# megvii-research/AAAI2023-PVD

Hardware: AMD Instinct MI355X
Metric: train rays/s (hash->vm chair distillation step) (higher is better)
Workload: dtype f16 tables+MLP (AMP, as the reference forces) / f32 marcher+compositor; 1 GPU; distill hash->vm, synthetic chair, synthetic cameras, stage 3 (rgb + feature/sigma/colour losses), 4096 rays/GPU/step, occupancy 128^3 5.0% occupied, max_steps 1024, teacher pre-trained 300 steps; rays_per_gpu=4096, parallelism=ray-dp1, update=AdamW in one launch, capture_fallback=False

## Files before the change

aaai2023-pvd_amd/csrc/raymarching.hip:

```cpp
#include "dda.h"
#include "rays.h"

#include <float.h>

namespace pvd {

constexpr uint32_t kBlock = 256;
constexpr float kRPi = 0.3183098861837907f;


__global__ void __launch_bounds__(kBlock) k_near_far(const float *__restrict__ rays_o, const float *__restrict__ rays_d,
                                                     const float *__restrict__ aabb, uint32_t N, float min_near,
                                                     float *__restrict__ nears, float *__restrict__ fars) {
    const uint32_t n = blockIdx.x * kBlock + threadIdx.x;
    if (n >= N) return;
    const float o[3] = {rays_o[3 * (size_t)n], rays_o[3 * (size_t)n + 1], rays_o[3 * (size_t)n + 2]};
    const float d[3] = {rays_d[3 * (size_t)n], rays_d[3 * (size_t)n + 1], rays_d[3 * (size_t)n + 2]};
    near_far_of(o, d, aabb, min_near, nears[n], fars[n]);
}

__global__ void __launch_bounds__(kBlock) k_polar(const float *__restrict__ rays_o, const float *__restrict__ rays_d,
                                                  float radius, uint32_t N, float *__restrict__ coords) {
    const uint32_t n = blockIdx.x * kBlock + threadIdx.x;
    if (n >= N) return;
    const float ox = rays_o[3 * (size_t)n], oy = rays_o[3 * (size_t)n + 1], oz = rays_o[3 * (size_t)n + 2];
    const float dx = rays_d[3 * (size_t)n], dy = rays_d[3 * (size_t)n + 1], dz = rays_d[3 * (size_t)n + 2];
    const float A = dx * dx + dy * dy + dz * dz;
    const float Bh = ox * dx + oy * dy + oz * dz;
    const float Cc = ox * ox + oy * oy + oz * oz - radius * radius;
    const float t = (-Bh + sqrtf(Bh * Bh - A * Cc)) / A;
    const float x = ox + t * dx, y = oy + t * dy, z = oz + t * dz;
    const float theta = atan2f(sqrtf(x * x + z * z), y);
    const float phi = atan2f(z, x);
    coords[2 * (size_t)n] = 2 * theta * kRPi - 1;
// ... 254 lines not shown
            const uint32_t n_before = emitted - (uint32_t)__popcll(emit_mask);
            const int prev_lane = below ? 63 - __clzll((long long)below) : 0;
            const float prev_after = __shfl(t_after, prev_lane, 64);
            if ((emit_mask >> lane) & 1ull) {
                const size_t k = n_before + (uint32_t)__popcll(below);
                xyzs[3 * k] = x; xyzs[3 * k + 1] = y; xyzs[3 * k + 2] = z;
                dirs[3 * k] = r.dx; dirs[3 * k + 1] = r.dy; dirs[3 * k + 2] = r.dz;
                deltas[2 * k] = dtp;
                deltas[2 * k + 1] = t_after - (below ? prev_after : last_t);
            }
            last_t = readlane_f(t_after, 63u - (uint32_t)__clzll((long long)emit_mask));
        }
        if (rec && emit_mask) {
            if (rec->n < kMarchMaxRecords) {
                if (lane == 0) { rec->chunk[rec->n].mask = emit_mask; rec->chunk[rec->n].t_base = t_base; }
                rec->n++;
            } else {
                rec->overflow = true;
            }
        }
        if (done) break;
        t_base = readlane_f(t_after, 63);
        if (!fast && !grows) {
            const uint32_t b61 = __float_as_uint(readlane_f(t_after, 61)), b62 = __float_as_uint(readlane_f(t_after, 62));
            const uint32_t b63 = __float_as_uint(t_base);
            lat_c = ((b61 >> 23) == (b63 >> 23) && (b62 >> 23) == (b63 >> 23)) ? b63 - b62 : 0u;
        }
    }
    return emitted;
}

constexpr uint32_t kRaysPerBlock = kBlock / kWave;

__global__ void __launch_bounds__(kBlock) k_march_count_wave(const float *__restrict__ rays_o, const float *__restrict__ rays_d,
                                                             const uint8_t *__restrict__ grid, float bound, float dt_gamma, uint32_t max_steps,
                                                             uint32_t N, uint32_t C, uint32_t H, const float *__restrict__ nears,
                                                             const float *__restrict__ fars, int32_t *__restrict__ rays, uint32_t perturb,
                                                             MarchRayRecords *__restrict__ records, const int32_t *__restrict__ counter,
                                                             uint32_t fresh) {
    if (records && blockIdx.x == 0 && threadIdx.x == 0) records[N].n = fresh ? 0u : (uint32_t)counter[0];
    const uint32_t n = blockIdx.x * kRaysPerBlock + (threadIdx.x >> 6);
    const uint32_t lane = threadIdx.x & 63u;
    if (n >= N) return;
#ifdef PVD_MARCH_PROFILE
    const long long prof_t0 = __builtin_readcyclecounter();
    uint32_t prof_chunks = 0;
#endif
    Dda r;
    r.init(rays_o + 3 * (size_t)n, rays_d + 3 * (size_t)n, bound, dt_gamma, max_steps, C, H, grid);
    const float t0 = ray_t0(nears[n], r.dt_min, perturb, 42u, n);
    const float far = fars[n];
    uint32_t num;
    if (t0 >= 0.0f && t0 < far) {
        MarchRecord rec = {records ? records[n].chunk : nullptr, 0u, false};
#ifdef PVD_MARCH_PROFILE
        num = march_ray_wave<false>(r, t0, far, max_steps, lane, nullptr, nullptr, nullptr, &prof_chunks, records ? &rec : nullptr);
#else
        num = march_ray_wave<false>(r, t0, far, max_steps, lane, nullptr, nullptr, nullptr, nullptr, records ? &rec : nullptr);
#endif
        if (records && lane == 0) { records[n].n = rec.n; records[n].overflow = rec.overflow ? 1u : 0u; }
    } else {
        float t = t0;
        num = 0;
        while (t < far && num < max_steps) {
            float x, y, z, dt, tn;
            if (r.probe(t, x, y, z, dt, tn)) { num++; t += dt; }
            else t = tn;
        }
        if (records && lane == 0) { records[n].n = 0; records[n].overflow = num ? 1u : 0u; }
    }
    if (lane == 0) rays[3 * (size_t)n + 2] = (int32_t)num;
#ifdef PVD_MARCH_PROFILE
    if (lane == 0) { rays[3 * (size_t)n] = (int32_t)(__builtin_readcyclecounter() - prof_t0); rays[3 * (size_t)n + 1] = (int32_t)prof_chunks; }
#endif
}

__global__ void __launch_bounds__(kBlock) k_march_write_wave(const float *__restrict__ rays_o, const float *__restrict__ rays_d,
                                                             const uint8_t *__restrict__ grid, float bound, float dt_gamma, uint32_t max_steps,
                                                             uint32_t N, uint32_t C, uint32_t H, uint32_t M,
                                                             const float *__restrict__ nears, const float *__restrict__ fars,
                                                             float *__restrict__ xyzs, float *__restrict__ dirs, float *__restrict__ deltas,
                                                             const int32_t *__restrict__ rays, uint32_t perturb,
                                                             const int32_t *__restrict__ budget) {
    const uint32_t n = blockIdx.x * kRaysPerBlock + (threadIdx.x >> 6);
    const uint32_t lane = threadIdx.x & 63u;
    if (n >= N) return;
// ... 672 lines not shown

int pvd_morton3D_invert(const int32_t *indices, uint32_t N, int32_t *coords, pvd_stream_t stream) {
    if (N == 0) return PVD_OK;
    PVD_REQUIRE(coords && indices);
    hipLaunchKernelGGL(k_morton3D_invert, dim3(div_up(N, kBlock)), dim3(kBlock), 0, (hipStream_t)stream, indices, N, coords);
    return check_launch();
}

int pvd_packbits(const float *grid, uint32_t N, float density_thresh, uint8_t *bitfield, pvd_stream_t stream) {
    if (N == 0) return PVD_OK;
    PVD_REQUIRE(grid && bitfield);
    PVD_REQUIRE((reinterpret_cast<uintptr_t>(grid) & 15u) == 0);
    hipLaunchKernelGGL(k_packbits, dim3(div_up(N, kBlock)), dim3(kBlock), 0, (hipStream_t)stream, grid, N, density_thresh, bitfield);
    return check_launch();
}

constexpr uint32_t kMarchFusedScanMaxRays = 16384;

size_t pvd_march_workspace_bytes(uint32_t N) { return ((size_t)N + 1) * sizeof(MarchRayRecords); }

int pvd_march_rays_train(const float *rays_o, const float *rays_d, const uint8_t *grid, float bound, float dt_gamma,
                         uint32_t max_steps, uint32_t N, uint32_t C, uint32_t H, uint32_t M, const float *nears,
                         const float *fars, float *xyzs, float *dirs, float *deltas, int32_t *rays, int32_t *counter,
                         uint32_t perturb, pvd_stream_t stream) {
    return pvd_march_rays_train_ws(rays_o, rays_d, grid, bound, dt_gamma, max_steps, N, C, H, M, nears, fars, xyzs, dirs, deltas, rays,
                                   counter, perturb, nullptr, 0, 0u, nullptr, stream);
}

int pvd_march_rays_train_ws(const float *rays_o, const float *rays_d, const uint8_t *grid, float bound, float dt_gamma,
                            uint32_t max_steps, uint32_t N, uint32_t C, uint32_t H, uint32_t M, const float *nears,
                            const float *fars, float *xyzs, float *dirs, float *deltas, int32_t *rays, int32_t *counter,
                            uint32_t perturb, void *workspace, size_t workspace_bytes, uint32_t flags, const int32_t *budget_dev,
                            pvd_stream_t stream) {
    hipStream_t s = (hipStream_t)stream;
    const bool fresh = (flags & PVD_MARCH_FRESH) != 0;
    if (N == 0) {
        if (fresh && M && xyzs && dirs && deltas && counter) {
            (void)hipMemsetAsync(xyzs, 0, 3 * (size_t)M * sizeof(float), s); (void)hipMemsetAsync(dirs, 0, 3 * (size_t)M * sizeof(float), s);
            (void)hipMemsetAsync(deltas, 0, 2 * (size_t)M * sizeof(float), s); (void)hipMemsetAsync(counter, 0, 2 * sizeof(int32_t), s);
        }
        return PVD_OK;
    }
    PVD_REQUIRE(rays_o && rays_d && grid && nears && fars && xyzs && dirs && deltas && rays && counter);
    PVD_REQUIRE(C >= 1 && C <= 16 && H >= 1 && H <= 1024 && max_steps >= 1);
    MarchRayRecords *records = (workspace && workspace_bytes >= pvd_march_workspace_bytes(N) && N <= kMarchFusedScanMaxRays)
                                   ? (MarchRayRecords *)workspace : nullptr;
    if (fresh && !records) {
        (void)hipMemsetAsync(xyzs, 0, 3 * (size_t)M * sizeof(float), s); (void)hipMemsetAsync(dirs, 0, 3 * (size_t)M * sizeof(float), s);
        (void)hipMemsetAsync(deltas, 0, 2 * (size_t)M * sizeof(float), s); (void)hipMemsetAsync(counter, 0, 2 * sizeof(int32_t), s);
    }
    const dim3 g(div_up(N, kRaysPerBlock)), b(kBlock);
    hipLaunchKernelGGL(k_march_count_wave, g, b, 0, s, rays_o, rays_d, grid, bound, dt_gamma, max_steps, N, C, H, nears, fars, rays, perturb,
                       records, counter, records && fresh ? 1u : 0u);
    if (records) {
        hipLaunchKernelGGL(k_march_write_records, g, b, 0, s, rays_o, rays_d, grid, bound, dt_gamma, max_steps, N, C, H, M, nears, fars, xyzs,
                           dirs, deltas, rays, perturb, records, counter, fresh ? 1u : 0u, budget_dev);
        return check_launch();
    }
#ifdef PVD_MARCH_PROFILE
    return check_launch();
#endif
    hipLaunchKernelGGL(k_march_scan, dim3(1), dim3(kScanBlock), 0, s, rays, N, counter);
    hipLaunchKernelGGL(k_march_write_wave, g, b, 0, s, rays_o, rays_d, grid, bound, dt_gamma, max_steps, N, C, H, M, nears, fars, xyzs, dirs,
                       deltas, rays, perturb, budget_dev);
    return check_launch();
}

int pvd_composite_rays_train_forward(const float *sigmas, const float *rgbs, const float *deltas, const int32_t *rays,
                                     uint32_t M, uint32_t N, float *weights_sum, float *depth, float *image,
                                     pvd_stream_t stream) {
    if (N == 0) return PVD_OK;
    PVD_REQUIRE(sigmas && rgbs && deltas && rays && weights_sum && depth && image);
    hipLaunchKernelGGL(k_composite_fwd_wave<false>, dim3(div_up(N, kBlock / kWave)), dim3(kBlock), 0, (hipStream_t)stream, sigmas, rgbs, deltas,
                       rays, M, N, weights_sum, depth, image, CompositeEpilogue{});
    return check_launch();
}

int pvd_composite_rays_train_backward(const float *grad_weights_sum, const float *grad_image, const float *sigmas,
                                      const float *rgbs, const float *deltas, const int32_t *rays, const float *weights_sum,
                                      const float *image, uint32_t M, uint32_t N, float *grad_sigmas, float *grad_rgbs,
                                      pvd_stream_t stream) {
    if (N == 0) return PVD_OK;
    PVD_REQUIRE(grad_weights_sum && grad_image && sigmas && rgbs && deltas && rays && weights_sum && image && grad_sigmas && grad_rgbs);
    hipLaunchKernelGGL(k_composite_bwd_wave<false>, dim3(div_up(N, kBlock / kWave)), dim3(kBlock), 0, (hipStream_t)stream, grad_weights_sum,
                       grad_image, sigmas, rgbs, deltas, rays, weights_sum, image, M, N, grad_sigmas, grad_rgbs, CompositeEpilogue{});
    return check_launch();
// ... 162 lines not shown
```

aaai2023-pvd_amd/pvd/renderer.py:

```python
import math

import numpy as np
import torch
import torch.nn as nn


def near_far_from_aabb_torch(rays_o, rays_d, aabb, min_near):
    rd = 1.0 / rays_d
    lo = (aabb[:3] - rays_o) * rd
    hi = (aabb[3:] - rays_o) * rd
    t_lo, t_hi = torch.minimum(lo, hi), torch.maximum(lo, hi)
    near, far = t_lo[:, 0], t_hi[:, 0]
    miss = torch.zeros_like(near, dtype=torch.bool)
    for a in (1, 2):
        miss = miss | (near > t_hi[:, a]) | (t_lo[:, a] > far)
        near, far = torch.maximum(near, t_lo[:, a]), torch.minimum(far, t_hi[:, a])
    big = torch.finfo(near.dtype).max
    near = torch.where(miss, torch.full_like(near, big), near.clamp_min(min_near))
    far = torch.where(miss, torch.full_like(far, big), far)
    return near, far


def sample_pdf(bins, weights, n_samples, det=False):
    pdf = weights + 1e-5
# ... 8 lines not shown
    hi = torch.searchsorted(cdf, u, right=True)
    lo = (hi - 1).clamp_min(0)
    hi = hi.clamp_max(cdf.shape[-1] - 1)
    c_lo, c_hi = torch.gather(cdf, -1, lo), torch.gather(cdf, -1, hi)
    b_lo, b_hi = torch.gather(bins, -1, lo), torch.gather(bins, -1, hi)
    width = c_hi - c_lo
    width = torch.where(width < 1e-5, torch.ones_like(width), width)
    return b_lo + (u - c_lo) / width * (b_hi - b_lo)


class NeRFRenderer(nn.Module):
    def __init__(self, ops, bound=1, cuda_ray=True, density_scale=1, min_near=0.2, density_thresh=0.01, bg_radius=-1,
                 grid_size=128, teacher_variant=False):
        super().__init__()
        self.ops = ops
        self.rm = ops.raymarching
        self.bound = bound
        self.cascade = 1 + math.ceil(math.log2(bound))
        self.grid_size = grid_size
        self.density_scale = density_scale
        self.min_near = min_near
        self.density_thresh = density_thresh
        self.bg_radius = bg_radius
        self.teacher_variant = teacher_variant

        aabb = torch.FloatTensor([-bound, -bound, -bound, bound, bound, bound])
        self.register_buffer("aabb_train", aabb)
        self.register_buffer("aabb_infer", aabb.clone())

        self.cuda_ray = cuda_ray
        if cuda_ray:
            self.register_buffer("density_grid", torch.zeros([self.cascade, grid_size ** 3]))
            self.register_buffer("density_bitfield", torch.zeros(self.cascade * grid_size ** 3 // 8, dtype=torch.uint8))
            self.mean_density = 0
            self.iter_density = 0
            self.register_buffer("step_counter", torch.zeros(16, 2, dtype=torch.int32))
            self.mean_count = 0
            self.local_step = 0
        if bg_radius > 0:
            raise NotImplementedError("bg_radius > 0 (background model) is not supported: the reference's own branch asserts out "
                                      "(distill_mutual/network.py:496)")
        self.occ_epoch = 0

    def note_occupancy_changed(self):
        self.occ_epoch += 1

    def load_state_dict(self, state_dict, strict=True, **kw):
        out = super().load_state_dict(state_dict, strict=strict, **kw)
        self.note_occupancy_changed()
        return out

    def forward(self, x, d):
        raise NotImplementedError()

    def density(self, x):
        raise NotImplementedError()

    def reset_extra_state(self):
        if not self.cuda_ray:
            return
        self.density_grid.zero_()
        self.note_occupancy_changed()
        self.mean_density = 0
        self.iter_density = 0
        self.step_counter.zero_()
        self.mean_count = 0
        self.local_step = 0

    def run(self, rays_o, rays_d, num_steps=128, upsample_steps=128, bg_color=None, perturb=False, **kwargs):
        prefix = rays_o.shape[:-1]
        rays_o = rays_o.contiguous().view(-1, 3)
        rays_d = rays_d.contiguous().view(-1, 3)
        N, device = rays_o.shape[0], rays_o.device
        aabb = self.aabb_train if self.training else self.aabb_infer
        nears, fars = near_far_from_aabb_torch(rays_o, rays_d, aabb, self.min_near)
        nears, fars = nears.unsqueeze(-1), fars.unsqueeze(-1)

        z_vals = nears + (fars - nears) * torch.linspace(0.0, 1.0, num_steps, device=device).unsqueeze(0)
# ... 49 lines not shown
        rm = self.rm
        prefix = rays_o.shape[:-1]
        rays_o = rays_o.contiguous().view(-1, 3)
        rays_d = rays_d.contiguous().view(-1, 3)
        N = rays_o.shape[0]
        device = rays_o.device

        nears_fars = kwargs.get("nears_fars")
        if nears_fars is not None:
            nears, fars = nears_fars
        else:
            nears, fars = rm.near_far_from_aabb(rays_o, rays_d, self.aabb_train if self.training else self.aabb_infer, self.min_near)

        if self.bg_radius > 0:
            polar = rm.polar_from_ray(rays_o, rays_d, self.bg_radius)
            bg_color = self.background(polar, rays_d)
        elif bg_color is None:
            bg_color = 1

        if self.training:
            stu_first = bool(getattr(self.args, "render_stu_first", True))
            i_march = (not self.is_teacher) if stu_first else self.is_teacher
            if self.teacher_variant:
                i_march = True
            premarched = kwargs.get("premarched", False)
            if premarched:
                i_march = False
            else:
                counter = self.step_counter[self.local_step % 16]
                self.local_step += 1
            budget = self._budget() if not force_all_rays else None
            own = i_march or bool(kwargs.get("own_march", False))
            if i_march:
                if budget is not None:
                    xyzs, dirs, deltas, rays = rm.march_rays_train(rays_o, rays_d, self.bound, self.density_bitfield, self.cascade,
                                                                   self.grid_size, nears, fars, counter, self.mean_count, perturb, 128,
                                                                   force_all_rays, dt_gamma, max_steps, True, budget)
                else:
                    xyzs, dirs, deltas, rays = rm.march_rays_train(rays_o, rays_d, self.bound, self.density_bitfield, self.cascade,
                                                                   self.grid_size, nears, fars, counter, self.mean_count, perturb, 128,
                                                                   force_all_rays, dt_gamma, max_steps, True)
                inherited_params = [xyzs, dirs, deltas, rays]
            else:
                xyzs, dirs, deltas, rays = inherited_params

            sigmas, rgbs = self(xyzs, dirs)

            if not self.teacher_variant:
                gs, st = self.args.global_step, self.args.stage_iters
                if gs < st["stage1"]:
                    return {"stage1": gs, "depth": None, "image": None, "inherited_params": inherited_params, "sigmas": sigmas, "rays": rays}
                if gs < st["stage2"]:
                    return {"stage2": gs, "depth": None, "image": None, "inherited_params": inherited_params, "sigmas": sigmas, "rays": rays}

            if self.density_scale != 1:
                sigmas = self.density_scale * sigmas
            eps = 0.0 if self.teacher_variant else 1e-6
            ride = kwargs.get("objective")
            if ride is not None and not (torch.is_grad_enabled() and ride.with_student(getattr(self, "feature_sigma_color", None), getattr(self, "color_l", None))):
                ride = None
            okw = {} if ride is None else {"objective": ride}
            if budget is not None and own:
                weights_sum, depth, image = rm.composite_rays_train_bg(sigmas, rgbs, deltas, rays, bg_color, nears, fars, eps, True, budget[1], **okw)
            else:
                weights_sum, depth, image = rm.composite_rays_train_bg(sigmas, rgbs, deltas, rays, bg_color, nears, fars, eps, True, **okw)
            image = image.view(*prefix, 3)
            depth = depth.view(*prefix)
            return {"depth": depth, "image": image, "inherited_params": inherited_params, "sigmas": sigmas, "rays": rays,
                    "nears_fars": (nears, fars)}

        if self._persistent_render(rays_o, perturb):
            if self.model_type == "tensors":
                run = self.ops.plenoxel.infer_image
            else:
# ... 72 lines not shown
        xyzs, dirs, deltas = torch.empty(rows, 3, **f32), torch.empty(rows, 3, **f32), torch.empty(rows, 2, **f32)
        rows_dev = state[4:5]
        n_upper, i = N, 0
        while True:
            for _ in range(check_every):
                cur, old = i & 1, (i & 1) ^ 1
                if i > 0:
                    rm.infer_compact(state, cur, n_upper, rays_alive[cur], rays_alive[old], rays_t[cur], rays_t[old])
                rm.infer_round_begin(state, cur, N, max_steps)
                rm.infer_march(state, n_upper, rays_alive[cur], rays_t[cur], rays_o, rays_d, self.bound, dt_gamma, max_steps, self.cascade,
                               self.grid_size, self.density_bitfield, fars, xyzs, dirs, deltas, False)
                m_upper = min(rows, 8 * n_upper + (128 - (8 * n_upper) % 128) % 128)
                sigmas, rgbs = self.forward_rows(xyzs[:m_upper], dirs[:m_upper], rows_dev)
                rm.infer_composite(state, n_upper, rays_alive[cur], rays_t[cur], sigmas, rgbs.float(), deltas, float(self.density_scale),
                                   weights_sum, depth, image)
                i += 1
            n_alive, steps_done = state[2:6:3].tolist()
            if n_alive <= 0 or steps_done >= max_steps:
                break
            n_upper = min(n_upper, n_alive)
        self._last_rounds = int(state[6])
        image = image + (1 - weights_sum).unsqueeze(-1) * bg_color
        depth = torch.clamp(depth - nears, min=0) / (fars - nears)
        return {"depth": depth.view(*prefix), "image": image.view(*prefix, 3), "inherited_params": inherited_params}

    def march(self, rays_o, rays_d, dt_gamma=0, perturb=False, force_all_rays=False, max_steps=1024, nears_fars=None):
        rm = self.rm
        rays_o = rays_o.contiguous().view(-1, 3)
        rays_d = rays_d.contiguous().view(-1, 3)
        nears, fars = nears_fars if nears_fars is not None else rm.near_far_from_aabb(rays_o, rays_d, self.aabb_train, self.min_near)
        counter = self.step_counter[self.local_step % 16]
        self.local_step += 1
        budget = self._budget() if not force_all_rays else None
        extra = (budget,) if budget is not None else ()
        xyzs, dirs, deltas, rays = rm.march_rays_train(rays_o, rays_d, self.bound, self.density_bitfield, self.cascade, self.grid_size,
                                                       nears, fars, counter, self.mean_count, perturb, 128, force_all_rays, dt_gamma,
                                                       max_steps, True, *extra)
        return [xyzs, dirs, deltas, rays], (nears, fars)

    def _cell_centres(self, coords, cas, jitter):
        H = self.grid_size
        xyzs = 2 * coords.float() / (H - 1) - 1
        bound = min(2 ** cas, self.bound)
        hgs = bound / H
        p = xyzs * (bound - hgs)
        if jitter:
            p = p + (torch.rand_like(p) * 2 - 1) * hgs
        return p, hgs

    @torch.no_grad()
    def mark_untrained_grid(self, poses, intrinsic, S=64):
        if not self.cuda_ray:
            return
        if isinstance(poses, np.ndarray):
            poses = torch.from_numpy(poses)
        dev = self.density_grid.device
        poses = poses.to(dev)
        B = poses.shape[0]
        fx, fy, cx, cy = intrinsic
        H = self.grid_size
        axis = torch.arange(H, dtype=torch.int32, device=dev)
        count = torch.zeros_like(self.density_grid)
        for xs in axis.split(S):
            for ys in axis.split(S):
                for zs in axis.split(S):
                    xx, yy, zz = torch.meshgrid(xs, ys, zs, indexing="ij")
                    coords = torch.stack([xx.reshape(-1), yy.reshape(-1), zz.reshape(-1)], dim=-1)
                    indices = self.rm.morton3D(coords).long()
                    for cas in range(self.cascade):
                        world, hgs = self._cell_centres(coords, cas, jitter=False)
                        for head in range(0, B, S):
# ... 170 lines not shown
```

aaai2023-pvd_amd/pvd_hip/__init__.py:

```python
import ctypes
import os
import sys
import types

_HWQ = "GPU_MAX_HW_QUEUES"
_torch_loaded = sys.modules.get("torch")
if _HWQ in os.environ:
    HW_QUEUES, HW_QUEUES_SOURCE = os.environ[_HWQ], "caller"
elif os.environ.get("PVD_HW_QUEUES", "") == "keep":
    HW_QUEUES, HW_QUEUES_SOURCE = None, "left to the runtime (PVD_HW_QUEUES=keep)"
elif _torch_loaded is not None and _torch_loaded.cuda.is_initialized():
    HW_QUEUES, HW_QUEUES_SOURCE = None, "runtime started before pvd_hip was imported"
else:
    os.environ[_HWQ] = "2"
    HW_QUEUES, HW_QUEUES_SOURCE = "2", "package default"

import torch


def forked_graphs_ok():
    force = os.environ.get("PVD_FORKED_GRAPHS")
    if force in ("0", "1"):
        return force == "1"
    try:
# ... 10 lines not shown
        "libpvd_hip.so not found at %s -- build it with `python -c 'import __graft_entry__ as g; g.build()'` "
        "or `make -C aaai2023-pvd_amd/csrc` (there is no CPU fallback)" % LIB_PATH
    )

_lib = ctypes.CDLL(LIB_PATH)
_lib.pvd_status_string.restype = ctypes.c_char_p
_lib.pvd_last_hip_error.restype = ctypes.c_char_p
_lib.pvd_abi_version.restype = ctypes.c_int

ABI_VERSION = int(_lib.pvd_abi_version())

_u32, _f32, _int, _vp = ctypes.c_uint32, ctypes.c_float, ctypes.c_int, ctypes.c_void_p

PVD_F32, PVD_F16 = 0, 1

ENTRY_POINTS = (
    "pvd_abi_version", "pvd_status_string", "pvd_last_hip_error",
    "pvd_near_far_from_aabb", "pvd_polar_from_ray", "pvd_morton3D", "pvd_morton3D_invert", "pvd_packbits",
    "pvd_march_rays_train", "pvd_march_rays_train_ws", "pvd_march_workspace_bytes", "pvd_composite_rays_train_forward", "pvd_composite_rays_train_backward",
    "pvd_march_rays", "pvd_composite_rays", "pvd_compact_rays", "pvd_infer_round_begin", "pvd_infer_compact", "pvd_infer_march", "pvd_infer_composite", "pvd_occ_sample", "pvd_occ_update", "pvd_occ_finish", "pvd_occ_sample_replay", "pvd_occ_update_ordered",
    "pvd_mse_forward", "pvd_grid_encode_forward", "pvd_grid_encode_forward_affine", "pvd_grid_encode_forward_affine_pack", "pvd_grid_encode_backward", "pvd_grid_encode_backward_affine",
    "pvd_sh_encode_forward", "pvd_sh_encode_backward",
    "pvd_vm_forward", "pvd_vm_forward_pack_rider", "pvd_vm_backward", "pvd_infer_image_vm", "pvd_infer_image_plenoxel", "pvd_vm_backward_rider", "pvd_head_backward_defer", "pvd_plenoxel_forward", "pvd_plenoxel_backward", "pvd_get_rays", "pvd_make_ray_batch",
    "pvd_head_forward", "pvd_hash_head_forward_fused", "pvd_hash_head_forward_fused_span", "pvd_infer_image_hash",
    "pvd_head_backward", "pvd_head_backward_workspace_floats", "pvd_head_image_halfs", "pvd_head_pack_weights",
    "pvd_composite_rays_train_bg_forward", "pvd_composite_rays_train_bg_backward",
    "pvd_composite_objective_blocks", "pvd_composite_objective_blocks_fixed", "pvd_composite_objective_forward", "pvd_composite_objective_backward",
    "pvd_distill_sumsq", "pvd_distill_loss_final", "pvd_distill_sumsq_backward", "pvd_distill_loss_backward", "pvd_grid_set_variant", "pvd_grid_set_fwd_kernel",
    "pvd_adamw_step", "pvd_adamw_step_ex", "pvd_adamw_lazy_flush", "pvd_freq_encode", "pvd_mlp_head_forward_fused", "pvd_check_finite", "pvd_check_finite_f16", "pvd_check_finite_mixed", "pvd_l1_ranges", "pvd_segments_op", "pvd_segments_gather_zero_check",
)
ENTRY_POINTS_MLP = ("pvd_mlp_head_forward_fused_rows", "pvd_infer_image_mlp")
ENTRY_POINTS_METRICS = ("pvd_image_metrics_workspace_floats", "pvd_image_metrics")
ENTRY_POINTS_DATA = ("pvd_image_batch", "pvd_error_map_update")
for _name in ENTRY_POINTS + ENTRY_POINTS_MLP + ENTRY_POINTS_METRICS + ENTRY_POINTS_DATA:
    if _name not in ("pvd_status_string", "pvd_last_hip_error"):
        getattr(_lib, _name).restype = ctypes.c_int
_lib.pvd_march_workspace_bytes.restype = ctypes.c_size_t
_lib.pvd_composite_objective_blocks.restype = ctypes.c_uint32
_lib.pvd_composite_objective_blocks_fixed.restype = ctypes.c_uint32


class PvdHipError(RuntimeError):
    pass


def _check(status, what):
    if status != 0:
        msg = _lib.pvd_status_string(status).decode()
        hip = _lib.pvd_last_hip_error().decode()
        raise PvdHipError("%s: %s%s" % (what, msg, (" [%s]" % hip) if hip else ""))


def _dev(*tensors):
    dev = None
    for t in tensors:
        if t is None:
            continue
        if not t.is_cuda:
            raise PvdHipError("tensor must be a CUDA(HIP) tensor -- libpvd_hip has no CPU path")
        if not t.is_contiguous():
            raise PvdHipError("tensor must be contiguous")
        if dev is None:
            dev = t.device
        elif t.device != dev:
            raise PvdHipError("all tensors must be on the same device")
    return dev

# ... 96 lines not shown
    if bg is not None:
        _want(bg, torch.float32, "bg")
    if state.numel() < 3:
        raise PvdHipError("state must hold 3 int64 values")
    _call("pvd_make_ray_batch", dev, _p(poses), _u32(poses.shape[0]), _p(state), ctypes.c_uint64(int(seed) & (2 ** 64 - 1)), _f32(fx),
          _f32(fy), _f32(cx), _f32(cy), _u32(H), _u32(W), _u32(N), _p(aabb), _f32(min_near), _p(inds), _p(rays_o), _p(rays_d), _p(bg),
          _p(nears), _p(fars))


def polar_from_ray(rays_o, rays_d, radius, N, coords):
    dev = _dev(rays_o, rays_d, coords)
    _f32_all(rays_o=rays_o, rays_d=rays_d, coords=coords)
    _call("pvd_polar_from_ray", dev, _p(rays_o), _p(rays_d), _f32(radius), _u32(N), _p(coords))


def morton3D(coords, N, indices):
    dev = _dev(coords, indices)
    _want(coords, torch.int32, "coords"), _want(indices, torch.int32, "indices")
    _call("pvd_morton3D", dev, _p(coords), _u32(N), _p(indices))


def morton3D_invert(indices, N, coords):
    dev = _dev(coords, indices)
    _want(coords, torch.int32, "coords"), _want(indices, torch.int32, "indices")
    _call("pvd_morton3D_invert", dev, _p(indices), _u32(N), _p(coords))


def packbits(grid, N, density_thresh, bitfield):
    dev = _dev(grid, bitfield)
    _want(grid, torch.float32, "grid"), _want(bitfield, torch.uint8, "bitfield")
    _call("pvd_packbits", dev, _p(grid), _u32(N), _f32(density_thresh), _p(bitfield))


def march_rays_train(rays_o, rays_d, grid, bound, dt_gamma, max_steps, N, C, H, M, nears, fars,
                     xyzs, dirs, deltas, rays, counter, perturb, use_workspace=True, fresh=False, budget_dev=None):
    dev = _dev(rays_o, rays_d, grid, nears, fars, xyzs, dirs, deltas, rays, counter, budget_dev)
    if budget_dev is not None:
        _want(budget_dev, torch.int32, "budget_dev")
    _f32_all(rays_o=rays_o, rays_d=rays_d, nears=nears, fars=fars, xyzs=xyzs, dirs=dirs, deltas=deltas)
    _want(grid, torch.uint8, "grid"), _want(rays, torch.int32, "rays"), _want(counter, torch.int32, "counter")
    ws = _march_workspace(dev, N) if use_workspace else None
    _call("pvd_march_rays_train_ws", dev, _p(rays_o), _p(rays_d), _p(grid), _f32(bound), _f32(dt_gamma), _u32(max_steps),
          _u32(N), _u32(C), _u32(H), _u32(M), _p(nears), _p(fars), _p(xyzs), _p(dirs), _p(deltas), _p(rays), _p(counter),
          _u32(int(perturb)), _p(ws), ctypes.c_size_t(ws.numel() if ws is not None else 0), _u32(1 if fresh else 0), _p(budget_dev))


MARCH_FRESH = True


_march_ws = {}


def _march_workspace(dev, N):
    if N > 16384:
        return None
    key = (dev, torch.cuda.current_stream(dev).cuda_stream, N)
    ws = _march_ws.get(key)
    if ws is None:
        ws = torch.empty(int(_lib.pvd_march_workspace_bytes(_u32(N))), dtype=torch.uint8, device=dev)
        _march_ws[key] = ws
    return ws


def composite_rays_train_forward(sigmas, rgbs, deltas, rays, M, N, weights_sum, depth, image):
    dev = _dev(sigmas, rgbs, deltas, rays, weights_sum, depth, image)
    _f32_all(sigmas=sigmas, rgbs=rgbs, deltas=deltas, weights_sum=weights_sum, depth=depth, image=image)
    _want(rays, torch.int32, "rays")
    _call("pvd_composite_rays_train_forward", dev, _p(sigmas), _p(rgbs), _p(deltas), _p(rays), _u32(M), _u32(N),
          _p(weights_sum), _p(depth), _p(image))


def composite_rays_train_backward(grad_weights_sum, grad_image, sigmas, rgbs, deltas, rays, weights_sum, image, M, N,
                                  grad_sigmas, grad_rgbs):
    dev = _dev(grad_weights_sum, grad_image, sigmas, rgbs, deltas, rays, weights_sum, image, grad_sigmas, grad_rgbs)
# ... 1031 lines not shown
            raise PvdHipError("inds_coarse must hold N cells when an error map is given")
        _want(inds_coarse, torch.int64, "inds_coarse")
        if keys_out is not None:
            _want(keys_out, torch.float32, "keys_out")
            if keys_out.numel() < g * g:
                raise PvdHipError("keys_out must hold g*g floats")
    _call("pvd_image_batch", dev, _p(images), _p(poses), _p(order), _u32(V), _u32(H), _u32(W), _u32(C), _p(state),
          ctypes.c_uint64(int(seed) & (2 ** 64 - 1)), _f32(fx), _f32(fy), _f32(cx), _f32(cy), _u32(N), _p(aabb), _f32(min_near),
          _p(error_map), _u32(g), _p(view_out), _p(inds), _p(inds_coarse if error_map is not None else None), _p(rays_o), _p(rays_d),
          _p(gt), _p(bg), _p(nears), _p(fars), _p(keys_out if error_map is not None else None))


def error_map_update(error_map, view, inds_coarse, pred, gt, N):
    dev = _dev(error_map, view, inds_coarse, pred, gt)
    _f32_all(error_map=error_map, pred=pred, gt=gt)
    _want(view, torch.int32, "view"), _want(inds_coarse, torch.int64, "inds_coarse")
    N = int(N)
    if error_map.dim() != 2:
        raise PvdHipError("error_map must be [V, g*g]")
    g = int(round(error_map.shape[1] ** 0.5))
    if g == 0 or g * g != error_map.shape[1]:
        raise PvdHipError("error_map must be [V, g*g]")
    if min(pred.numel(), gt.numel()) < 3 * N or inds_coarse.numel() < N or view.numel() < 1:
        raise PvdHipError("view [1], inds_coarse [N], pred and gt [N,3] are needed")
    _call("pvd_error_map_update", dev, _p(error_map), _u32(g), _p(view), _p(inds_coarse), _p(pred), _p(gt), _u32(N))


raymarching_backend = types.SimpleNamespace(
    composite_rays_train_bg_forward=composite_rays_train_bg_forward, composite_rays_train_bg_backward=composite_rays_train_bg_backward,
    composite_objective_forward=composite_objective_forward, composite_objective_backward=composite_objective_backward,
    composite_objective_blocks=composite_objective_blocks,
    get_rays=get_rays, near_far_from_aabb=near_far_from_aabb, polar_from_ray=polar_from_ray, morton3D=morton3D,
    morton3D_invert=morton3D_invert, packbits=packbits, march_rays_train=march_rays_train,
    composite_rays_train_forward=composite_rays_train_forward,
    composite_rays_train_backward=composite_rays_train_backward,
    march_rays=march_rays, composite_rays=composite_rays, compact_rays=compact_rays, MARCH_FRESH=MARCH_FRESH,
    infer_round_begin=infer_round_begin, infer_compact=infer_compact, infer_march=infer_march, infer_composite=infer_composite,
    INFER_STATE_INTS=INFER_STATE_INTS,
)
gridencoder_backend = types.SimpleNamespace(grid_encode_forward=grid_encode_forward, grid_encode_backward=grid_encode_backward)
shencoder_backend = types.SimpleNamespace(sh_encode_forward=sh_encode_forward, sh_encode_backward=sh_encode_backward)
```

aaai2023-pvd_amd/raymarching/__init__.py:

```python
from pvd_hip import raymarching_backend as _backend

from .raymarching import make_ops

_ops = make_ops(_backend, device_type="cuda")

near_far_from_aabb = _ops.near_far_from_aabb
polar_from_ray = _ops.polar_from_ray
morton3D = _ops.morton3D
morton3D_invert = _ops.morton3D_invert
packbits = _ops.packbits
march_rays_train = _ops.march_rays_train
composite_rays_train = _ops.composite_rays_train
composite_rays_train_bg = _ops.composite_rays_train_bg
march_rays = _ops.march_rays
composite_rays = _ops.composite_rays
compact_rays = _ops.compact_rays

infer_round_begin, infer_compact, infer_march, infer_composite = _ops.infer_round_begin, _ops.infer_compact, _ops.infer_march, _ops.infer_composite
INFER_STATE_INTS = _ops.INFER_STATE_INTS
```

aaai2023-pvd_amd/raymarching/raymarching.py:

```python
import types

import torch
from torch.autograd import Function
from torch.amp import custom_bwd, custom_fwd


def make_ops(backend, device_type="cuda"):
    fwd32 = custom_fwd(device_type=device_type, cast_inputs=torch.float32)
    bwd = custom_bwd(device_type=device_type)

    def _to_dev(t):
        if device_type == "cuda" and not t.is_cuda:
            return t.cuda()
        return t

    class _NearFar(Function):
        @staticmethod
        @fwd32
        def forward(ctx, rays_o, rays_d, aabb, min_near=0.2):
            rays_o = _to_dev(rays_o).contiguous().view(-1, 3)
            rays_d = _to_dev(rays_d).contiguous().view(-1, 3)
            N = rays_o.shape[0]
            nears = torch.empty(N, dtype=rays_o.dtype, device=rays_o.device)
            fars = torch.empty(N, dtype=rays_o.dtype, device=rays_o.device)
# ... 15 lines not shown
        @staticmethod
        def forward(ctx, coords):
            coords = _to_dev(coords)
            N = coords.shape[0]
            indices = torch.empty(N, dtype=torch.int32, device=coords.device)
            backend.morton3D(coords.int().contiguous(), N, indices)
            return indices

    class _MortonInvert(Function):
        @staticmethod
        def forward(ctx, indices):
            indices = _to_dev(indices)
            N = indices.shape[0]
            coords = torch.empty(N, 3, dtype=torch.int32, device=indices.device)
            backend.morton3D_invert(indices.int().contiguous(), N, coords)
            return coords

    class _Packbits(Function):
        @staticmethod
        @fwd32
        def forward(ctx, grid, thresh, bitfield=None):
            grid = _to_dev(grid).contiguous()
            C, H3 = grid.shape[0], grid.shape[1]
            N = C * H3 // 8
            if bitfield is None:
                bitfield = torch.empty(N, dtype=torch.uint8, device=grid.device)
            backend.packbits(grid, N, thresh, bitfield)
            return bitfield

    class _MarchTrain(Function):
        @staticmethod
        @fwd32
        def forward(ctx, rays_o, rays_d, bound, density_bitfield, C, H, nears, fars, step_counter=None, mean_count=-1,
                    perturb=False, align=-1, force_all_rays=False, dt_gamma=0, max_steps=1024, scratch_counter=False, budget=None):
            rays_o = _to_dev(rays_o).contiguous().view(-1, 3)
            rays_d = _to_dev(rays_d).contiguous().view(-1, 3)
            density_bitfield = _to_dev(density_bitfield).contiguous()
            N = rays_o.shape[0]
            M = N * max_steps
            if not force_all_rays and mean_count > 0:
                if align > 0:
                    mean_count += align - mean_count % align
                M = mean_count
            budget_dev = None
            if budget is not None and not force_all_rays and mean_count > 0:
                M, budget_dev = int(budget[0]), budget[1]
                assert M >= 1 and hasattr(backend, "MARCH_FRESH"), "a device-side budget needs the HIP backend"
            dev, dt = rays_o.device, rays_o.dtype
            fresh = bool(getattr(backend, "MARCH_FRESH", False)) and (scratch_counter or step_counter is None)
            alloc = torch.empty if fresh else torch.zeros
            buf = alloc(M * 8, dtype=dt, device=dev)
            xyzs, dirs, deltas = buf[:3 * M].view(M, 3), buf[3 * M:6 * M].view(M, 3), buf[6 * M:].view(M, 2)
            rays = torch.empty(N, 3, dtype=torch.int32, device=dev)
            if step_counter is None:
                step_counter = alloc(2, dtype=torch.int32, device=dev)
            elif scratch_counter and not fresh:
                step_counter.zero_()
            if budget_dev is not None:
                backend.march_rays_train(rays_o, rays_d, density_bitfield, bound, dt_gamma, max_steps, N, C, H, M, nears, fars,
                                         xyzs, dirs, deltas, rays, step_counter, perturb, fresh=fresh, budget_dev=budget_dev)
            elif fresh:
                backend.march_rays_train(rays_o, rays_d, density_bitfield, bound, dt_gamma, max_steps, N, C, H, M, nears, fars,
                                         xyzs, dirs, deltas, rays, step_counter, perturb, fresh=True)
            else:
                backend.march_rays_train(rays_o, rays_d, density_bitfield, bound, dt_gamma, max_steps, N, C, H, M, nears, fars,
                                         xyzs, dirs, deltas, rays, step_counter, perturb)
            if force_all_rays or mean_count <= 0:
                m = step_counter[0].item()
                if align > 0:
                    m += align - m % align
                xyzs, dirs, deltas = xyzs[:m], dirs[:m], deltas[:m]
                if device_type == "cuda":
                    torch.cuda.empty_cache()
            return xyzs, dirs, deltas, rays

    class _CompositeTrain(Function):
        @staticmethod
        @fwd32
        def forward(ctx, sigmas, rgbs, deltas, rays):
            sigmas = sigmas.contiguous()
            rgbs = rgbs.contiguous()
            M, N = sigmas.shape[0], rays.shape[0]
            weights_sum = torch.empty(N, dtype=sigmas.dtype, device=sigmas.device)
            depth = torch.empty(N, dtype=sigmas.dtype, device=sigmas.device)
            image = torch.empty(N, 3, dtype=sigmas.dtype, device=sigmas.device)
            backend.composite_rays_train_forward(sigmas, rgbs, deltas, rays, M, N, weights_sum, depth, image)
            ctx.save_for_backward(sigmas, rgbs, deltas, rays, weights_sum, depth, image)
            ctx.dims = [M, N]
            return weights_sum, depth, image

        @staticmethod
        @bwd
        def backward(ctx, grad_weights_sum, grad_depth, grad_image):
            grad_weights_sum = grad_weights_sum.contiguous()
            grad_image = grad_image.contiguous()
            sigmas, rgbs, deltas, rays, weights_sum, depth, image = ctx.saved_tensors
            M, N = ctx.dims
            gbuf = torch.zeros(sigmas.shape[0] * 4, dtype=sigmas.dtype, device=sigmas.device)
            grad_sigmas, grad_rgbs = gbuf[:sigmas.shape[0]], gbuf[sigmas.shape[0]:].view(-1, 3)
# ... 79 lines not shown
    class _March(Function):
        @staticmethod
        @fwd32
        def forward(ctx, n_alive, n_step, rays_alive, rays_t, rays_o, rays_d, bound, density_bitfield, C, H, near, far,
                    align=-1, perturb=False, dt_gamma=0, max_steps=1024):
            rays_o = _to_dev(rays_o).contiguous().view(-1, 3)
            rays_d = _to_dev(rays_d).contiguous().view(-1, 3)
            M = n_alive * n_step
            if align > 0:
                M += align - (M % align)
            dev, dt = rays_o.device, rays_o.dtype
            xyzs = torch.zeros(M, 3, dtype=dt, device=dev)
            dirs = torch.zeros(M, 3, dtype=dt, device=dev)
            deltas = torch.zeros(M, 2, dtype=dt, device=dev)
            backend.march_rays(n_alive, n_step, rays_alive, rays_t, rays_o, rays_d, bound, dt_gamma, max_steps, C, H,
                               density_bitfield, near, far, xyzs, dirs, deltas, perturb)
            return xyzs, dirs, deltas

    class _Composite(Function):
        @staticmethod
        @fwd32
        def forward(ctx, n_alive, n_step, rays_alive, rays_t, sigmas, rgbs, deltas, weights_sum, depth, image):
            backend.composite_rays(n_alive, n_step, rays_alive, rays_t, sigmas, rgbs, deltas, weights_sum, depth, image)
            return tuple()

    class _Compact(Function):
        @staticmethod
        @fwd32
        def forward(ctx, n_alive, rays_alive, rays_alive_old, rays_t, rays_t_old, alive_counter):
            backend.compact_rays(n_alive, rays_alive, rays_alive_old, rays_t, rays_t_old, alive_counter)
            return tuple()

    extra = {}
    if hasattr(backend, "infer_march"):
        extra = dict(infer_round_begin=backend.infer_round_begin, infer_compact=backend.infer_compact, infer_march=backend.infer_march,
                     infer_composite=backend.infer_composite, INFER_STATE_INTS=backend.INFER_STATE_INTS)
    return types.SimpleNamespace(
        **extra,
        near_far_from_aabb=_NearFar.apply,
        polar_from_ray=_Polar.apply,
        morton3D=_Morton.apply,
        morton3D_invert=_MortonInvert.apply,
        packbits=_Packbits.apply,
        march_rays_train=_MarchTrain.apply,
        composite_rays_train=_CompositeTrain.apply,
        composite_rays_train_bg=composite_rays_train_bg,
        march_rays=_March.apply,
        composite_rays=_Composite.apply,
        compact_rays=_Compact.apply,
    )
```

Before: 11.37 million rays/s.

## Add coarse 8^3 occupancy mask to skip and trim empty ray spans in marching

Builds a dilated coarse occupancy mask (one byte per 8^3 block, per cascade) from the density bitfield whenever occupancy changes. The training march kernel samples 64 points along each ray across its wave, skips rays whose samples all land in empty blocks, and otherwise shortens far to just past the last occupied sample. This targets the cost of DDA-stepping through empty space at 5% occupancy. It adds a small mask-build kernel and per-ray probe work, and relies on a conservative dilation margin to avoid dropping real samples.

```diff
diff --git a/aaai2023-pvd_amd/csrc/raymarching.hip b/aaai2023-pvd_amd/csrc/raymarching.hip
--- a/aaai2023-pvd_amd/csrc/raymarching.hip
+++ b/aaai2023-pvd_amd/csrc/raymarching.hip
@@ -1,5 +1,6 @@
 #include "dda.h"
 #include "rays.h"
+#include "../../include/pvd_hip_march.h"
 
 #include <float.h>
 
@@ -320,12 +321,77 @@
 
 constexpr uint32_t kRaysPerBlock = kBlock / kWave;
 
+constexpr uint32_t kCoarseShift = 3;
+static_assert((1u << kCoarseShift) == PVD_COARSE_BLOCK, "coarse block edge");
+
+__global__ void __launch_bounds__(kBlock) k_occ_coarse_mask(const uint8_t *__restrict__ bitfield, uint32_t C, uint32_t H,
+                                                            uint8_t *__restrict__ mask) {
+    const uint32_t G = H >> kCoarseShift, G3 = G * G * G;
+    const uint32_t i = blockIdx.x * kBlock + threadIdx.x;
+    if (i >= C * G3) return;
+    const uint32_t c = i / G3, b = i - c * G3;
+    const uint32_t bx = b / (G * G), by = (b / G) % G, bz = b % G;
+    const uint8_t *cascade = bitfield + (size_t)c * ((size_t)H * H * H / 8);
+    uint32_t any = 0;
+    for (uint32_t x = max(bx, 1u) - 1u; x <= min(bx + 1u, G - 1u); x++)
+        for (uint32_t y = max(by, 1u) - 1u; y <= min(by + 1u, G - 1u); y++)
+            for (uint32_t z = max(bz, 1u) - 1u; z <= min(bz + 1u, G - 1u); z++) {
+                const uint4 *p = reinterpret_cast<const uint4 *>(cascade + (size_t)morton3(x, y, z) * 64u);
+#pragma unroll
+                for (int q = 0; q < 4; q++) { const uint4 v = p[q]; any |= v.x | v.y | v.z | v.w; }
+            }
+    mask[i] = any ? (uint8_t)1 : (uint8_t)0;
+}
+
+__device__ __forceinline__ bool coarse_confine(const Dda &r, const uint8_t *__restrict__ mask, float t0, float &far, uint32_t lane,
+                                               bool &empty) {
+    empty = false;
+    if (!mask || r.dt_gamma != 0.0f) return false;
+    const float span = far - t0;
+    if (!(span >= far * (1.0f / 1024.0f)) || !(span > 1e-6f)) return false;
+    const float step = span * (1.0f / 63.0f);
+    const float dmax = fmaxf(fabsf(r.dx), fmaxf(fabsf(r.dy), fabsf(r.dz)));
+    const float delta = 1.25f * (0.5f * step * dmax) + r.bound * (1.0f / 1048576.0f);
+    const float edge0 = (float)(2u << kCoarseShift) * r.mip_bound0 * r.rH;
+    if (!(delta <= 0.9f * edge0)) return false;
+
+    const float s = fmaf((float)lane, step, t0);
+    const float x = clampf(fmaf(s, r.dx, r.ox), -r.bound, r.bound);
+    const float y = clampf(fmaf(s, r.dy, r.oy), -r.bound, r.bound);
+    const float z = clampf(fmaf(s, r.dz, r.oz), -r.bound, r.bound);
+    int lo = 0, hi = 0;
+    if (!r.one_cascade) {
+        const float mx = fmaxf(fabsf(x), fmaxf(fabsf(y), fabsf(z)));
+        int e_lo, e_hi, e_dt;
+        (void)frexpf(fmaxf(mx - delta, 0.0f), &e_lo);
+        (void)frexpf(mx + delta, &e_hi);
+        (void)frexpf((float)((double)(r.dt_const * r.Hf) * 0.5), &e_dt);
+        const int lvl_dt = (int)fminf(r.Cf - 1, fmaxf(0.0f, (float)e_dt));
+        lo = max((int)fminf(r.Cf - 1, fmaxf(0.0f, (float)e_lo)), lvl_dt);
+        hi = max((int)fminf(r.Cf - 1, fmaxf(0.0f, (float)e_hi)), lvl_dt);
+    }
+    const uint32_t G = r.H >> kCoarseShift;
+    bool hit = false;
+    for (int level = lo; level <= hi; level++) {
+        const float mip_rbound = 1.0f / fminf((float)(1 << level), r.bound);
+        const uint32_t bx = (uint32_t)(int)clampf(fmaf(x, mip_rbound, 1.0f) * r.half_h, 0.0f, r.cell_hi) >> kCoarseShift;
+        const uint32_t by = (uint32_t)(int)clampf(fmaf(y, mip_rbound, 1.0f) * r.half_h, 0.0f, r.cell_hi) >> kCoarseShift;
+        const uint32_t bz = (uint32_t)(int)clampf(fmaf(z, mip_rbound, 1.0f) * r.half_h, 0.0f, r.cell_hi) >> kCoarseShift;
+        hit = hit || mask[(size_t)level * G * G * G + (bx * G + by) * G + bz] != 0;
+    }
+    const uint64_t hits = __ballot(hit);
+    if (hits == 0) { empty = true; return true; }
+    const uint32_t last = 63u - (uint32_t)__clzll((long long)hits);
+    if (last < 63u) far = fminf(far, fmaf((float)(last + 1u), step, t0));
+    return true;
+}
+
 __global__ void __launch_bounds__(kBlock) k_march_count_wave(const float *__restrict__ rays_o, const float *__restrict__ rays_d,
                                                              const uint8_t *__restrict__ grid, float bound, float dt_gamma, uint32_t max_steps,
                                                              uint32_t N, uint32_t C, uint32_t H, const float *__restrict__ nears,
                                                              const float *__restrict__ fars, int32_t *__restrict__ rays, uint32_t perturb,
                                                              MarchRayRecords *__restrict__ records, const int32_t *__restrict__ counter,
-                                                             uint32_t fresh) {
+                                                             uint32_t fresh, const uint8_t *__restrict__ coarse_mask) {
     if (records && blockIdx.x == 0 && threadIdx.x == 0) records[N].n = fresh ? 0u : (uint32_t)counter[0];
     const uint32_t n = blockIdx.x * kRaysPerBlock + (threadIdx.x >> 6);
     const uint32_t lane = threadIdx.x & 63u;
@@ -337,9 +403,13 @@
     Dda r;
     r.init(rays_o + 3 * (size_t)n, rays_d + 3 * (size_t)n, bound, dt_gamma, max_steps, C, H, grid);
     const float t0 = ray_t0(nears[n], r.dt_min, perturb, 42u, n);
-    const float far = fars[n];
+    float far = fars[n];
     uint32_t num;
-    if (t0 >= 0.0f && t0 < far) {
+    bool empty = false;
+    if (t0 >= 0.0f && t0 < far && coarse_confine(r, coarse_mask, t0, far, lane, empty) && empty) {
+        num = 0;
+        if (records && lane == 0) { records[n].n = 0; records[n].overflow = 0u; }
+    } else if (t0 >= 0.0f && t0 < far) {
         MarchRecord rec = {records ? records[n].chunk : nullptr, 0u, false};
 #ifdef PVD_MARCH_PROFILE
         num = march_ray_wave<false>(r, t0, far, max_steps, lane, nullptr, nullptr, nullptr, &prof_chunks, records ? &rec : nullptr);
@@ -1078,6 +1148,24 @@
                             const float *fars, float *xyzs, float *dirs, float *deltas, int32_t *rays, int32_t *counter,
                             uint32_t perturb, void *workspace, size_t workspace_bytes, uint32_t flags, const int32_t *budget_dev,
                             pvd_stream_t stream) {
+    return pvd_march_rays_train_mask(rays_o, rays_d, grid, bound, dt_gamma, max_steps, N, C, H, M, nears, fars, xyzs, dirs, deltas, rays,
+                                     counter, perturb, workspace, workspace_bytes, flags, budget_dev, nullptr, stream);
+}
+
+int pvd_occ_coarse_mask(const uint8_t *bitfield, uint32_t C, uint32_t H, uint8_t *mask, pvd_stream_t stream) {
+    PVD_REQUIRE(bitfield && mask && C >= 1 && C <= 16 && H >= 1 && H <= 1024);
+    if ((H & (H - 1u)) || H < PVD_COARSE_BLOCK) return PVD_ERR_UNSUPPORTED;
+    PVD_REQUIRE((reinterpret_cast<uintptr_t>(bitfield) & 15u) == 0);
+    const uint32_t G = H >> kCoarseShift;
+    hipLaunchKernelGGL(k_occ_coarse_mask, dim3(div_up(C * G * G * G, kBlock)), dim3(kBlock), 0, (hipStream_t)stream, bitfield, C, H, mask);
+    return check_launch();
+}
+
+int pvd_march_rays_train_mask(const float *rays_o, const float *rays_d, const uint8_t *grid, float bound, float dt_gamma,
+                              uint32_t max_steps, uint32_t N, uint32_t C, uint32_t H, uint32_t M, const float *nears,
+                              const float *fars, float *xyzs, float *dirs, float *deltas, int32_t *rays, int32_t *counter,
+                              uint32_t perturb, void *workspace, size_t workspace_bytes, uint32_t flags,
+                              const int32_t *budget_dev, const uint8_t *coarse_mask, pvd_stream_t stream) {
     hipStream_t s = (hipStream_t)stream;
     const bool fresh = (flags & PVD_MARCH_FRESH) != 0;
     if (N == 0) {
@@ -1096,8 +1184,9 @@
         (void)hipMemsetAsync(deltas, 0, 2 * (size_t)M * sizeof(float), s); (void)hipMemsetAsync(counter, 0, 2 * sizeof(int32_t), s);
     }
     const dim3 g(div_up(N, kRaysPerBlock)), b(kBlock);
+    if ((H & (H - 1u)) || H < PVD_COARSE_BLOCK) coarse_mask = nullptr;
     hipLaunchKernelGGL(k_march_count_wave, g, b, 0, s, rays_o, rays_d, grid, bound, dt_gamma, max_steps, N, C, H, nears, fars, rays, perturb,
-                       records, counter, records && fresh ? 1u : 0u);
+                       records, counter, records && fresh ? 1u : 0u, coarse_mask);
     if (records) {
         hipLaunchKernelGGL(k_march_write_records, g, b, 0, s, rays_o, rays_d, grid, bound, dt_gamma, max_steps, N, C, H, M, nears, fars, xyzs,
                            dirs, deltas, rays, perturb, records, counter, fresh ? 1u : 0u, budget_dev);
diff --git a/aaai2023-pvd_amd/pvd/renderer.py b/aaai2023-pvd_amd/pvd/renderer.py
--- a/aaai2023-pvd_amd/pvd/renderer.py
+++ b/aaai2023-pvd_amd/pvd/renderer.py
@@ -64,6 +64,9 @@
         if cuda_ray:
             self.register_buffer("density_grid", torch.zeros([self.cascade, grid_size ** 3]))
             self.register_buffer("density_bitfield", torch.zeros(self.cascade * grid_size ** 3 // 8, dtype=torch.uint8))
+            n_coarse = self.cascade * (grid_size // 8) ** 3 if grid_size >= 8 and grid_size & (grid_size - 1) == 0 else 0
+            self.register_buffer("density_coarse_mask", torch.zeros(n_coarse, dtype=torch.uint8), persistent=False)
+            self._coarse_mask_key = None
             self.mean_density = 0
             self.iter_density = 0
             self.register_buffer("step_counter", torch.zeros(16, 2, dtype=torch.int32))
@@ -76,6 +79,20 @@
 
     def note_occupancy_changed(self):
         self.occ_epoch += 1
+        if self.cuda_ray:
+            self._coarse_mask_key = None
+            self.coarse_mask()
+
+    def coarse_mask(self):
+        build = getattr(self.rm, "occ_coarse_mask", None)
+        mask, bits = self.density_coarse_mask, self.density_bitfield
+        if build is None or mask.numel() == 0 or not (bits.is_cuda and mask.is_cuda):
+            return None
+        key = (bits.data_ptr(), bits._version, mask.data_ptr())
+        if key != self._coarse_mask_key:
+            build(bits, self.cascade, self.grid_size, mask)
+            self._coarse_mask_key = key
+        return mask
 
     def load_state_dict(self, state_dict, strict=True, **kw):
         out = super().load_state_dict(state_dict, strict=strict, **kw)
@@ -191,14 +208,8 @@
             budget = self._budget() if not force_all_rays else None
             own = i_march or bool(kwargs.get("own_march", False))
             if i_march:
-                if budget is not None:
-                    xyzs, dirs, deltas, rays = rm.march_rays_train(rays_o, rays_d, self.bound, self.density_bitfield, self.cascade,
-                                                                   self.grid_size, nears, fars, counter, self.mean_count, perturb, 128,
-                                                                   force_all_rays, dt_gamma, max_steps, True, budget)
-                else:
-                    xyzs, dirs, deltas, rays = rm.march_rays_train(rays_o, rays_d, self.bound, self.density_bitfield, self.cascade,
-                                                                   self.grid_size, nears, fars, counter, self.mean_count, perturb, 128,
-                                                                   force_all_rays, dt_gamma, max_steps, True)
+                xyzs, dirs, deltas, rays = self._march_train(rays_o, rays_d, nears, fars, counter, perturb, force_all_rays, dt_gamma,
+                                                             max_steps, budget)
                 inherited_params = [xyzs, dirs, deltas, rays]
             else:
                 xyzs, dirs, deltas, rays = inherited_params
@@ -337,11 +348,14 @@
         counter = self.step_counter[self.local_step % 16]
         self.local_step += 1
         budget = self._budget() if not force_all_rays else None
-        extra = (budget,) if budget is not None else ()
-        xyzs, dirs, deltas, rays = rm.march_rays_train(rays_o, rays_d, self.bound, self.density_bitfield, self.cascade, self.grid_size,
-                                                       nears, fars, counter, self.mean_count, perturb, 128, force_all_rays, dt_gamma,
-                                                       max_steps, True, *extra)
+        xyzs, dirs, deltas, rays = self._march_train(rays_o, rays_d, nears, fars, counter, perturb, force_all_rays, dt_gamma, max_steps, budget)
         return [xyzs, dirs, deltas, rays], (nears, fars)
+
+    def _march_train(self, rays_o, rays_d, nears, fars, counter, perturb, force_all_rays, dt_gamma, max_steps, budget):
+        coarse = self.coarse_mask()
+        extra = () if budget is None and coarse is None else (budget,) if coarse is None else (budget, coarse)
+        return self.rm.march_rays_train(rays_o, rays_d, self.bound, self.density_bitfield, self.cascade, self.grid_size, nears, fars,
+                                        counter, self.mean_count, perturb, 128, force_all_rays, dt_gamma, max_steps, True, *extra)
 
     def _cell_centres(self, coords, cas, jitter):
         H = self.grid_size
diff --git a/aaai2023-pvd_amd/pvd_hip/__init__.py b/aaai2023-pvd_amd/pvd_hip/__init__.py
--- a/aaai2023-pvd_amd/pvd_hip/__init__.py
+++ b/aaai2023-pvd_amd/pvd_hip/__init__.py
@@ -66,7 +66,8 @@
 ENTRY_POINTS_MLP = ("pvd_mlp_head_forward_fused_rows", "pvd_infer_image_mlp")
 ENTRY_POINTS_METRICS = ("pvd_image_metrics_workspace_floats", "pvd_image_metrics")
 ENTRY_POINTS_DATA = ("pvd_image_batch", "pvd_error_map_update")
-for _name in ENTRY_POINTS + ENTRY_POINTS_MLP + ENTRY_POINTS_METRICS + ENTRY_POINTS_DATA:
+ENTRY_POINTS_MARCH = ("pvd_occ_coarse_mask", "pvd_march_rays_train_mask")
+for _name in ENTRY_POINTS + ENTRY_POINTS_MLP + ENTRY_POINTS_METRICS + ENTRY_POINTS_DATA + ENTRY_POINTS_MARCH:
     if _name not in ("pvd_status_string", "pvd_last_hip_error"):
         getattr(_lib, _name).restype = ctypes.c_int
 _lib.pvd_march_workspace_bytes.restype = ctypes.c_size_t
@@ -229,14 +230,41 @@
     _call("pvd_packbits", dev, _p(grid), _u32(N), _f32(density_thresh), _p(bitfield))
 
 
+COARSE_BLOCK = 8
+
+
+def coarse_mask_bytes(C, H):
+    C, H = int(C), int(H)
+    return C * (H // COARSE_BLOCK) ** 3 if H >= COARSE_BLOCK and H & (H - 1) == 0 else 0
+
+
+def occ_coarse_mask(bitfield, C, H, mask):
+    dev = _dev(bitfield, mask)
+    _want(bitfield, torch.uint8, "bitfield"), _want(mask, torch.uint8, "mask")
+    C, H = int(C), int(H)
+    if coarse_mask_bytes(C, H) == 0 or mask.numel() != coarse_mask_bytes(C, H) or bitfield.numel() != C * H ** 3 // 8:
+        raise PvdHipError("mask must hold C * (H/8)^3 bytes and bitfield C * H^3 / 8 (H a power of two >= 8)")
+    _call("pvd_occ_coarse_mask", dev, _p(bitfield), _u32(C), _u32(H), _p(mask))
+
+
 def march_rays_train(rays_o, rays_d, grid, bound, dt_gamma, max_steps, N, C, H, M, nears, fars,
-                     xyzs, dirs, deltas, rays, counter, perturb, use_workspace=True, fresh=False, budget_dev=None):
-    dev = _dev(rays_o, rays_d, grid, nears, fars, xyzs, dirs, deltas, rays, counter, budget_dev)
+                     xyzs, dirs, deltas, rays, counter, perturb, use_workspace=True, fresh=False, budget_dev=None, coarse_mask=None):
+    dev = _dev(rays_o, rays_d, grid, nears, fars, xyzs, dirs, deltas, rays, counter, budget_dev, coarse_mask)
+    if coarse_mask is not None:
+        _want(coarse_mask, torch.uint8, "coarse_mask")
+        if coarse_mask.numel() != coarse_mask_bytes(C, H):
+            raise PvdHipError("coarse_mask must hold C * (H/8)^3 bytes")
     if budget_dev is not None:
         _want(budget_dev, torch.int32, "budget_dev")
     _f32_all(rays_o=rays_o, rays_d=rays_d, nears=nears, fars=fars, xyzs=xyzs, dirs=dirs, deltas=deltas)
     _want(grid, torch.uint8, "grid"), _want(rays, torch.int32, "rays"), _want(counter, torch.int32, "counter")
     ws = _march_workspace(dev, N) if use_workspace else None
+    if coarse_mask is not None:
+        _call("pvd_march_rays_train_mask", dev, _p(rays_o), _p(rays_d), _p(grid), _f32(bound), _f32(dt_gamma), _u32(max_steps),
+              _u32(N), _u32(C), _u32(H), _u32(M), _p(nears), _p(fars), _p(xyzs), _p(dirs), _p(deltas), _p(rays), _p(counter),
+              _u32(int(perturb)), _p(ws), ctypes.c_size_t(ws.numel() if ws is not None else 0), _u32(1 if fresh else 0), _p(budget_dev),
+              _p(coarse_mask))
+        return
     _call("pvd_march_rays_train_ws", dev, _p(rays_o), _p(rays_d), _p(grid), _f32(bound), _f32(dt_gamma), _u32(max_steps),
           _u32(N), _u32(C), _u32(H), _u32(M), _p(nears), _p(fars), _p(xyzs), _p(dirs), _p(deltas), _p(rays), _p(counter),
           _u32(int(perturb)), _p(ws), ctypes.c_size_t(ws.numel() if ws is not None else 0), _u32(1 if fresh else 0), _p(budget_dev))
@@ -1334,6 +1362,7 @@
     composite_objective_blocks=composite_objective_blocks,
     get_rays=get_rays, near_far_from_aabb=near_far_from_aabb, polar_from_ray=polar_from_ray, morton3D=morton3D,
     morton3D_invert=morton3D_invert, packbits=packbits, march_rays_train=march_rays_train,
+    occ_coarse_mask=occ_coarse_mask, coarse_mask_bytes=coarse_mask_bytes,
     composite_rays_train_forward=composite_rays_train_forward,
     composite_rays_train_backward=composite_rays_train_backward,
     march_rays=march_rays, composite_rays=composite_rays, compact_rays=compact_rays, MARCH_FRESH=MARCH_FRESH,
diff --git a/aaai2023-pvd_amd/raymarching/__init__.py b/aaai2023-pvd_amd/raymarching/__init__.py
--- a/aaai2023-pvd_amd/raymarching/__init__.py
+++ b/aaai2023-pvd_amd/raymarching/__init__.py
@@ -18,3 +18,5 @@
 
 infer_round_begin, infer_compact, infer_march, infer_composite = _ops.infer_round_begin, _ops.infer_compact, _ops.infer_march, _ops.infer_composite
 INFER_STATE_INTS = _ops.INFER_STATE_INTS
+
+occ_coarse_mask, coarse_mask_bytes = _ops.occ_coarse_mask, _ops.coarse_mask_bytes
diff --git a/aaai2023-pvd_amd/raymarching/raymarching.py b/aaai2023-pvd_amd/raymarching/raymarching.py
--- a/aaai2023-pvd_amd/raymarching/raymarching.py
+++ b/aaai2023-pvd_amd/raymarching/raymarching.py
@@ -71,7 +71,8 @@
         @staticmethod
         @fwd32
         def forward(ctx, rays_o, rays_d, bound, density_bitfield, C, H, nears, fars, step_counter=None, mean_count=-1,
-                    perturb=False, align=-1, force_all_rays=False, dt_gamma=0, max_steps=1024, scratch_counter=False, budget=None):
+                    perturb=False, align=-1, force_all_rays=False, dt_gamma=0, max_steps=1024, scratch_counter=False, budget=None,
+                    coarse_mask=None):
             rays_o = _to_dev(rays_o).contiguous().view(-1, 3)
             rays_d = _to_dev(rays_d).contiguous().view(-1, 3)
             density_bitfield = _to_dev(density_bitfield).contiguous()
@@ -95,15 +96,16 @@
                 step_counter = alloc(2, dtype=torch.int32, device=dev)
             elif scratch_counter and not fresh:
                 step_counter.zero_()
+            ext = {}
+            if fresh:
+                ext["fresh"] = True
             if budget_dev is not None:
-                backend.march_rays_train(rays_o, rays_d, density_bitfield, bound, dt_gamma, max_steps, N, C, H, M, nears, fars,
-                                         xyzs, dirs, deltas, rays, step_counter, perturb, fresh=fresh, budget_dev=budget_dev)
-            elif fresh:
-                backend.march_rays_train(rays_o, rays_d, density_bitfield, bound, dt_gamma, max_steps, N, C, H, M, nears, fars,
-                                         xyzs, dirs, deltas, rays, step_counter, perturb, fresh=True)
-            else:
-                backend.march_rays_train(rays_o, rays_d, density_bitfield, bound, dt_gamma, max_steps, N, C, H, M, nears, fars,
-                                         xyzs, dirs, deltas, rays, step_counter, perturb)
+                ext["budget_dev"] = budget_dev
+            if coarse_mask is not None:
+                assert hasattr(backend, "occ_coarse_mask"), "a coarse occupancy mask needs the HIP backend"
+                ext["coarse_mask"] = coarse_mask
+            backend.march_rays_train(rays_o, rays_d, density_bitfield, bound, dt_gamma, max_steps, N, C, H, M, nears, fars,
+                                     xyzs, dirs, deltas, rays, step_counter, perturb, **ext)
             if force_all_rays or mean_count <= 0:
                 m = step_counter[0].item()
                 if align > 0:
@@ -249,8 +251,10 @@
             return tuple()
 
     extra = {}
+    if hasattr(backend, "occ_coarse_mask"):
+        extra.update(occ_coarse_mask=backend.occ_coarse_mask, coarse_mask_bytes=backend.coarse_mask_bytes)
     if hasattr(backend, "infer_march"):
-        extra = dict(infer_round_begin=backend.infer_round_begin, infer_compact=backend.infer_compact, infer_march=backend.infer_march,
+        extra.update(infer_round_begin=backend.infer_round_begin, infer_compact=backend.infer_compact, infer_march=backend.infer_march,
                      infer_composite=backend.infer_composite, INFER_STATE_INTS=backend.INFER_STATE_INTS)
     return types.SimpleNamespace(
         **extra,
diff --git a/include/pvd_hip_march.h b/include/pvd_hip_march.h
--- /dev/null
+++ b/include/pvd_hip_march.h
@@ -0,0 +1,24 @@
+#ifndef PVD_HIP_MARCH_H
+#define PVD_HIP_MARCH_H
+
+#include "pvd_hip.h"
+
+#ifdef __cplusplus
+extern "C" {
+#endif
+
+#define PVD_COARSE_BLOCK 8
+
+int pvd_occ_coarse_mask(const uint8_t *bitfield, uint32_t C, uint32_t H, uint8_t *mask, pvd_stream_t stream);
+
+int pvd_march_rays_train_mask(const float *rays_o, const float *rays_d, const uint8_t *grid, float bound, float dt_gamma,
+                              uint32_t max_steps, uint32_t N, uint32_t C, uint32_t H, uint32_t M, const float *nears,
+                              const float *fars, float *xyzs, float *dirs, float *deltas, int32_t *rays, int32_t *counter,
+                              uint32_t perturb, void *workspace, size_t workspace_bytes, uint32_t flags,
+                              const int32_t *budget_dev, const uint8_t *coarse_mask, pvd_stream_t stream);
+
+#ifdef __cplusplus
+}
+#endif
+
+#endif
```

After: 11.63 million rays/s (median of 6 runs). +2.3%, better.
